# maua-maua-maua/maua

Hardware: AMD Instinct MI355X
Metric: frames/sec (whole node), 1024x1024 StyleGAN2 audio-reactive render (higher is better)
Workload: dtype bf16

## Files before the change

maua_amd/csrc/internal.h:

```cpp
#pragma once
#include "common.h"

namespace maua {

int launch_pack_rgb8(hipStream_t stream, const float* img, uint8_t* out, int B, int H, int W);
template <typename TI, typename TO>
int launch_nchw_to_nhwc(hipStream_t s, const void* x, void* y, int N, int C, int HW, int Cp);
template <typename TI, typename TO>
int launch_nhwc_to_nchw(hipStream_t s, const void* x, void* y, int N, int C, int HW, int Cp);

struct ConvArgs {
  const void* x;
  long x_bstride;
  const void* w;
  const float* s;
  const float* d;
  const float* noise;
  long noise_bstride;
  float noise_strength;
  const float* noise_scale;
  const float* bias;
  void* y;
  int B, H, W, Ci, Co, up;
  int act;
// ... 80 lines not shown
size_t upwalk_weight_elems(int Co, int Ci);
int launch_upwalk(hipStream_t stream, const HiresArgs& a, int dtype = MAUA_BF16);
int launch_prep_upwalk_weights(hipStream_t stream, const float* w, void* wt, int Co, int Ci, int flip, int dtype = MAUA_BF16);
bool upwalk_fused_supported(int dtype, int Ci, int Cm, int H, int W);
int launch_upwalk_fused(hipStream_t stream, const HiresArgs& up, const HiresArgs& c1, int force_segs = 0, int narrow_ok = 1,
                        int dtype = MAUA_BF16);

int launch_prep_weights(hipStream_t stream, int dtype, const float* w, void* wt, float* wsq, int Co, int Ci, int k,
                        int up, int flip, int Cop, int Cip);
int launch_f32_split_inplace(hipStream_t stream, void* w, long n_floats);

int launch_tconv2(hipStream_t stream, int dtype, const ConvArgs& a);
bool tconv_dma_supported(int dtype, int Ci, int Co, int H, int W);
int launch_tconv_dma(hipStream_t stream, const ConvArgs& a, int dtype = MAUA_BF16);
int launch_tconv_edges(hipStream_t stream, const ConvArgs& a, int dtype = MAUA_BF16);
int launch_prep_tconv_weights(hipStream_t stream, int dtype, const float* w, void* wt, int Co, int Ci, int flip);

struct UpfirArgs {
  const void* t;
  void* y;
  const float* d;
  const float* noise;
  long noise_bstride;
  float noise_strength;
  const float* noise_scale;
  const float* bias;
  const float* out_scale;
  int B, H, W, Co;
  int act;
  float alpha, gain, clamp;
};
int launch_upfir_epilogue(hipStream_t stream, int dtype, const UpfirArgs& a);
bool tconv_fir_supported(int dtype, int Ci, int Co, int H, int W);
int launch_tconv_fir(hipStream_t stream, const ConvArgs& a, const UpfirArgs& u, int dtype = MAUA_BF16);
size_t prepped_weight_elems(int k, int up, int Cop, int Cip);

struct LayerOperands { const void* x; const void* w; const float* s; const float* d; const float* bias; void* y; int B, H, W, Ci, Co, up; };
struct NoiseOperands { const float* noise; long bstride; float strength; const float* scale; };
struct Epilogue { int act; float alpha, gain, clamp; };
template <typename A>
inline void set_noise_args(A& a, const NoiseOperands& n) {
  a.noise = n.noise; a.noise_bstride = n.bstride; a.noise_strength = n.strength; a.noise_scale = n.scale;
}
template <typename A>
inline void set_epilogue_args(A& a, const Epilogue& e) {
  a.act = e.act; a.alpha = e.alpha; a.gain = e.gain; a.clamp = e.clamp;
}
template <typename A>
inline A layer_args(A a, const LayerOperands& l, const NoiseOperands& n, const Epilogue& e) {
  a.x = l.x; a.w = l.w; a.s = l.s; a.d = l.d; a.bias = l.bias; a.y = l.y;
  a.B = l.B; a.H = l.H; a.W = l.W; a.Ci = l.Ci; a.Co = l.Co; a.up = l.up;
  set_noise_args(a, n);
  set_epilogue_args(a, e);
  return a;
}
template <typename A>
inline void fuse_torgb_args(A& a, const float* wmod, const float* bias, const float* prev, float* out, float clamp, const float* fir16) {
  a.rgb_wmod = wmod; a.rgb_bias = bias; a.rgb_prev = prev; a.rgb_out = out; a.rgb_clamp = clamp;
  for (int i = 0; i < 16; i++) a.fir[i] = fir16[i];
}
inline void pack_u8_args(HiresArgs& a, uint8_t* rgb8_out, bool skip_f32) {
  a.rgb8_out = rgb8_out;
  a.rgb_skip_f32 = skip_f32;
}
inline ConvArgs tconv_args(const void* x, long x_bstride, const void* w, const float* s, void* t, int B, int H, int W, int Ci, int Co) {
  ConvArgs a{};
  a.x = x; a.x_bstride = x_bstride; a.w = w; a.s = s; a.y = t;
  a.B = B; a.H = H; a.W = W; a.Ci = Ci; a.Co = Co; a.up = 2;
  return a;
}
inline UpfirArgs upfir_args(void* y, const float* d, const float* bias, const float* out_scale, int B, int H, int W, int Co,
                            const NoiseOperands& n, const Epilogue& e) {
  UpfirArgs u{};
  u.y = y; u.d = d; u.bias = bias; u.out_scale = out_scale; u.B = B; u.H = H; u.W = W; u.Co = Co;
  set_noise_args(u, n);
  set_epilogue_args(u, e);
  return u;
}
inline void upsample_fir16(float* fir) {
  const float g4[4] = {0.25f, 0.75f, 0.75f, 0.25f};
  for (int u = 0; u < 4; u++)
    for (int v = 0; v < 4; v++) fir[u * 4 + v] = g4[u] * g4[v];
}

int modconv3x3_check(int dtype, const ConvArgs& a);
int lowres_check(int dtype, const ConvArgs& a);
int lowres_ksplit(int dtype, int B, int H, int W, int Ci, int Co, int up);
int hires_check(const HiresArgs& a, int dtype);
int upwalk_check(const HiresArgs& a, int dtype);
int upwalk_fused_check(const HiresArgs& up, const HiresArgs& c1, int dtype);
int tconv2_check(int dtype, const ConvArgs& a);
int tconv_edges_check(const ConvArgs& a, int dtype);
int tconv_dma_check(const ConvArgs& a, int dtype);
int tconv_fir_check(const ConvArgs& a, const UpfirArgs& u, int dtype);
int upfir_check(int dtype, const UpfirArgs& a);

struct ResizeArgs {
  const void* x;
  long x_bstride;
  void* y;
  int B, H, W, C, oh, ow;
  int mode;
  int align;
  int pl, pt;
  int how;
  float value;
  const float* noise;
};
int launch_resize2d(hipStream_t stream, int dtype, bool nhwc, const ResizeArgs& a);
int launch_skip_add(hipStream_t stream, const float* y, const float* prev, float* out, int B, int H, int W,
                    const float* fir16);
int launch_warp_affine_nhwc(hipStream_t stream, int dtype, const void* x, void* y, const float* minv, int B, int H, int W,
                            int C);

struct StyleLayer {
  const float* affine_w;
  const float* affine_b;
  const float* wsq;
  const float* wrgb;
  float* s;
  float* d;
  float* wmod;
  int w_index;
  int Cin, Co, Cs, Cd;
  float scale;
};
int launch_styles(hipStream_t stream, const StyleLayer* layers_dev, int n_layers, const float* ws, int num_ws,
// ... 172 lines not shown
```

maua_amd/csrc/modconv_api.hip:

```cpp
#include <algorithm>
#include <cstring>

#include "common.h"
#include "internal.h"

namespace maua {
namespace {

enum { R_LOWRES = 0, R_GENERIC, R_DMA, R_HIRES, R_UPWALK, R_FUSED, R_WALKDONE, R_TFIR, R_TDMA, R_T2, R_UPFIR };

bool is_tconv(int r) { return r == R_TFIR || r == R_TDMA || r == R_T2; }
bool reads_premod(int r) { return r == R_TFIR || r == R_TDMA || r == R_DMA; }

LayerOperands operands(const maua_modconv_desc* d) {
  return LayerOperands{d->x, nullptr, d->s, d->d, d->bias, d->y, d->B, d->H, d->W, d->Ci, d->Co, d->up};
}
NoiseOperands noise_of(const maua_modconv_desc* d) { return NoiseOperands{d->noise, d->noise_bstride, d->noise_strength, d->noise_scale}; }
Epilogue epilogue_of(const maua_modconv_desc* d) { return Epilogue{d->act, d->alpha, d->gain, d->clamp}; }

template <typename A>
A desc_args(const maua_modconv_desc* d) {
  A a = layer_args(A{}, operands(d), noise_of(d), epilogue_of(d));
  if (d->rgb_out) {
    float fir[16];
// ... 160 lines not shown
    MAUA_HIP_CHECK(hipGetLastError());
  }
  switch (route) {
    case R_LOWRES:
    case R_GENERIC:
    case R_DMA: {
      ConvArgs a = conv_args(d);
      a.x = x; a.x_bstride = x_bstride; a.w = base + o_w;
      if (route == R_DMA) a.s = nullptr;
      return route == R_LOWRES    ? launch_modconv_lowres(st, dtype, a, base + o_xm, (float*)(base + o_ws))
             : route == R_GENERIC ? launch_modconv3x3(st, dtype, a)
                                  : launch_modconv_dma(st, a, dtype);
    }
    case R_HIRES:
    case R_UPWALK:
    case R_FUSED: {
      HiresArgs a = hires_args(d);
      a.w = base + o_w;
      if (route == R_HIRES) return launch_modconv_hires(st, a, dtype);
      if (route == R_UPWALK) return launch_upwalk(st, a, dtype);
      HiresArgs f = hires_args(d1);
      f.x = nullptr; f.y = nullptr; f.w = base + o_w1;
      a.y = nullptr;
      return launch_upwalk_fused(st, a, f, force_segs, narrow_ok, dtype);
    }
    case R_TFIR:
    case R_TDMA:
    case R_T2: {
      void* t = d->t ? d->t : base + o_t;
      ConvArgs a = tconv_args(d);
      a.x = x; a.x_bstride = x_bstride; a.w = base + o_w; a.y = t;
      if (route != R_T2) a.s = (const float*)(base + o_ones);
      UpfirArgs u = upfir_args(d);
      if (route == R_TFIR) return launch_tconv_fir(st, a, u, dtype);
      if (route == R_TDMA) {
        if (int rc = launch_tconv_edges(st, a, dtype)) return rc;
        if (int rc = launch_tconv_dma(st, a, dtype)) return rc;
      } else if (int rc = launch_tconv2(st, dtype, a)) {
        return rc;
      }
      u.t = t;
      return launch_upfir_epilogue(st, dtype, u);
    }
    case R_UPFIR: {
      UpfirArgs u = upfir_args(d);
      u.t = d->x;
      return launch_upfir_epilogue(st, dtype, u);
    }
  }
  return MAUA_OK;
}

extern "C" int maua_torgb_ex(maua_ctx* ctx, const void* x, const float* wmod, const float* bias, const float* prev, float* out, int B,
                             int H, int W, int C, float clamp, int dtype) {
  MAUA_REQUIRE(ctx && x && wmod && bias && out, "maua_torgb_ex: NULL argument");
  MAUA_REQUIRE(B >= 0 && H > 0 && W > 0 && C > 0, "maua_torgb_ex: bad shape");
  MAUA_REQUIRE(!prev || (H % 2 == 0 && W % 2 == 0), "maua_torgb_ex: the skip image needs an even grid");
  RgbArgs r{};
  r.x = x; r.wmod = wmod; r.bias = bias; r.prev = prev; r.out = out; r.B = B; r.H = H; r.W = W; r.C = C; r.clamp = clamp;
  upsample_fir16(r.fir);
  return launch_torgb(ctx->stream, dtype, r);
}
```

maua_amd/csrc/modconv_tconv_fir.hip:

```cpp
#include "common.h"
#include "internal.h"

namespace maua {

namespace {

constexpr int PTW = 32;
constexpr int HW1 = PTW + 1;
constexpr int KB = 64;
constexpr int WROWS = 9 * 32;
constexpr int WBUF = WROWS * KB;
constexpr int OFF_H = 2 * WBUF;
constexpr int ES = 128 * 2;

__device__ __constant__ const int kSlotF[9] = {0, 1, 1, 2, 2, 3, 3, 3, 3};
__device__ __constant__ const int kClsF[9] = {0, 0, 1, 0, 2, 0, 1, 2, 3};

__device__ __forceinline__ unsigned lds_off(const void* p) {
  return (unsigned)(size_t)(__attribute__((address_space(3))) const void*)p;
}
__device__ __forceinline__ void dma16_s(const void* sbase, unsigned voff, unsigned lds_dst) {
  asm volatile("s_mov_b32 m0, %2\n\ts_nop 0\n\tglobal_load_lds_dwordx4 %0, %1" ::"v"(voff), "s"(sbase), "s"(lds_dst)
               : "memory");
}
template <typename F>
__device__ __forceinline__ void mma(f32x16& acc, const u32x4& w, const u32x4& x) {
  Mma16<F>::step(acc, w, x);
}
__device__ __forceinline__ int swz(int n) { return (n >> 2) & 3; }

__device__ __forceinline__ int t_col(int tc, int pc) {
  const int p = tc >> 1;
  return p * ES + ((((tc & 1) ^ (p & 3)) << 6) | ((pc ^ ((p >> 2) & 3)) << 4));
}

template <typename F>
__device__ __forceinline__ void fir_hrow(const char* tile, int tr, const int (&tcol)[5], f32x2_t (&h)[2][4]) {
  f32x2_t c[5][4];
  const int rowb = (tr >> 1) * (PTW * ES), rsw = (tr & 1) << 7;
#pragma unroll
  for (int rx = 0; rx < 5; rx++) {
    const u32x4 v = *reinterpret_cast<const u32x4*>(tile + rowb + (tcol[rx] ^ rsw));
#pragma unroll
    for (int k = 0; k < 4; k++) c[rx][k] = f32x2_t{Fmt16<F>::lo(v[k]), Fmt16<F>::hi(v[k])};
  }
#pragma unroll
  for (int e = 0; e < 4; e++) {
    h[0][e] = (c[0][e] + c[3][e]) + 3.f * (c[1][e] + c[2][e]);
    h[1][e] = (c[1][e] + c[4][e]) + 3.f * (c[2][e] + c[3][e]);
  }
}

}

template <int PTH_, typename F>
__global__ __launch_bounds__(PTH_ * 32, PTH_ == 8 ? 2 : 1) void tconv_fir_kernel(ConvArgs a, UpfirArgs u) {
  constexpr int PTH = PTH_, UPR = PTH - 2;
  constexpr int HPX = (PTH + 1) * HW1, HBUF = HPX * KB;
  constexpr int NW = PTH / 2, NT = NW * 64;
  constexpr int WJ = (WBUF / 1024 + NW - 1) / NW, HJ = (HPX * 4 + NT - 1) / NT;
  constexpr int FG = NT / 128, FROWS = 2 * UPR / FG;
  static_assert(FG * FROWS == 2 * UPR, "output rows must split evenly over the FIR groups");
  extern __shared__ __attribute__((aligned(1024))) char smem[];
  const unsigned lds0 = __builtin_amdgcn_readfirstlane(lds_off(smem));
  const int tid = threadIdx.x, lane = tid & 63;
  const int wave = __builtin_amdgcn_readfirstlane(tid >> 6);
  const int r = lane & 31, h = lane >> 5;
  const int tiles_x = (a.W + 29) / 30, tiles = tiles_x * ((a.H + UPR - 1) / UPR), CB = a.Co >> 5;
  const int cbg = CB < 8 ? CB : 8, n_ts = tiles * a.B, per_group = ((n_ts + 7) >> 3) * 8 * cbg;
  const int L = blockIdx.x, grp = L / per_group, Lg = L - grp * per_group;
  const int xcd = Lg & 7, idx = Lg >> 3;
  const int cb = grp * cbg + idx % cbg, ts = (idx / cbg) * 8 + xcd;
  if (ts >= n_ts) return;
  const int b = ts / tiles, tile = ts - b * tiles;
  const int tyi = tile / tiles_x, txi = tile - tyi * tiles_x;
  const int ty0 = tyi * UPR - 1, tx0 = txi * 30 - 1;
  const char* xb = reinterpret_cast<const char*>(a.x) + (long)b * a.x_bstride * 2;
  const char* wp = reinterpret_cast<const char*>(a.w);

  unsigned hoff[HJ];
#pragma unroll
  for (int j = 0; j < HJ; j++) {
    const int P = (wave + NW * j) * 64 + lane;
    const int hp = P >> 2, q = (P & 3) ^ swz(hp);
    const int py = (hp * 1986) >> 16;
    const int px = hp - py * HW1;
    const int gy = ty0 - 1 + py, gx = tx0 - 1 + px;
    hoff[j] = 0xffffffffu;
    if (P < HPX * 4) {
      if (gy >= 0 && gx >= 0 && gy < a.H && gx < a.W) {
        hoff[j] = (unsigned)(((gy * a.W + gx) * a.Ci + q * 8) * 2);
      } else {
        *reinterpret_cast<u32x4*>(smem + OFF_H + P * 16) = u32x4{0u, 0u, 0u, 0u};
        *reinterpret_cast<u32x4*>(smem + OFF_H + HBUF + P * 16) = u32x4{0u, 0u, 0u, 0u};
      }
    }
  }
  unsigned woff[WJ];
#pragma unroll
  for (int j = 0; j < WJ; j++) {
    const int ii = wave + NW * j;
    const int R = min(16 * ii + (lane >> 2), WROWS - 1);
    const int k = R >> 5, n = R & 31;
    const int q = (lane & 3) ^ swz(R);
    woff[j] = (unsigned)((((((kSlotF[k] * CB + cb) * 4 + kClsF[k]) * 32 + n) * a.Ci) + q * 8) * 2);
  }
#define TD_ISSUE(C_, BUF_)                                                                               \
  {                                                                                                      \
    const char* ws_ = wp + (long)(C_) * KB;                                                              \
    _Pragma("unroll") for (int j = 0; j < WJ; j++)                                                      \
      if (wave + NW * j < WBUF / 1024) dma16_s(ws_, woff[j], lds0 + (BUF_) * WBUF + (wave + NW * j) * 1024); \
    const char* xs_ = xb + (long)(C_) * KB;                                                              \
    _Pragma("unroll") for (int j = 0; j < HJ; j++)                                                      \
      if (hoff[j] != 0xffffffffu) dma16_s(xs_, hoff[j], lds0 + OFF_H + (BUF_) * HBUF + (wave + NW * j) * 1024); \
  }

  const int hp00 = (2 * wave) * HW1 + r;
  const unsigned b0 = (unsigned)(r * KB + ((swz(r) ^ h) << 4));
#define TD_A(HR_, Q1_, KS_, BUF_)                                                                        \
  ({                                                                                                     \
    const int hp_ = hpv + (HR_) * HW1 + (Q1_);                                                           \
    *reinterpret_cast<const u32x4*>(smem + ((OFF_H + (BUF_) * HBUF + hp_ * KB + ((swz(hp_) ^ h) << 4)) ^ ((KS_) << 5))); \
  })
#define TD_B(K_, KS_, BUF_) (*reinterpret_cast<const u32x4*>(smem + (BUF_) * WBUF + (K_) * 32 * KB + (b0 ^ ((KS_) << 5))))

  f32x16 acc[2][4];
#pragma unroll
  for (int R = 0; R < 2; R++)
#pragma unroll
    for (int c = 0; c < 4; c++)
#pragma unroll
      for (int e = 0; e < 16; e++) acc[R][c][e] = 0.f;

  const int n_chunks = a.Ci >> 5;
  TD_ISSUE(0, 0)
  if (n_chunks > 1) TD_ISSUE(1, 1)
  asm volatile("s_waitcnt vmcnt(0)" ::: "memory");
  __syncthreads();
  int hpv = hp00;
#define TD_STEP(KS_, BUF_)                                                                               \
  {                                                                                                      \
    u32x4 A00 = TD_A(0, 0, KS_, BUF_), A01 = TD_A(0, 1, KS_, BUF_);      \
    u32x4 A10 = TD_A(1, 0, KS_, BUF_), A11 = TD_A(1, 1, KS_, BUF_);                    \
    u32x4 A20 = TD_A(2, 0, KS_, BUF_), A21 = TD_A(2, 1, KS_, BUF_);                    \
    {                                                                                                    \
      const u32x4 B0 = TD_B(0, KS_, BUF_), B1 = TD_B(1, KS_, BUF_), B2 = TD_B(2, KS_, BUF_);              \
      mma<F>(acc[0][0], B0, A00); mma<F>(acc[1][0], B0, A10);                                 \
      mma<F>(acc[0][1], B2, A01); mma<F>(acc[1][1], B2, A11);                        \
      mma<F>(acc[0][0], B1, A01); mma<F>(acc[1][0], B1, A11);                        \
    }                                                                                                    \
    {                                                                                                    \
      const u32x4 B3 = TD_B(3, KS_, BUF_), B4 = TD_B(4, KS_, BUF_);                                       \
      mma<F>(acc[0][2], B4, A10); mma<F>(acc[1][2], B4, A20);                        \
      mma<F>(acc[0][0], B3, A10); mma<F>(acc[1][0], B3, A20);                        \
    }                                                                                                    \
    {                                                                                                    \
      const u32x4 B5 = TD_B(5, KS_, BUF_), B6 = TD_B(6, KS_, BUF_), B7 = TD_B(7, KS_, BUF_), B8 = TD_B(8, KS_, BUF_); \
      mma<F>(acc[0][3], B8, A11); mma<F>(acc[1][3], B8, A21);                                 \
      mma<F>(acc[0][1], B6, A11); mma<F>(acc[1][1], B6, A21);                                                  \
      mma<F>(acc[0][2], B7, A11); mma<F>(acc[1][2], B7, A21);                                                  \
      mma<F>(acc[0][0], B5, A11); mma<F>(acc[1][0], B5, A21);                                                  \
    }                                                                                                    \
  }
  for (int c = 0; c < n_chunks; c++) {
    const int buf = c & 1;
    asm volatile("" : "+v"(hpv));
    TD_STEP(0, buf)
    {
      u32x4 A00 = TD_A(0, 0, 1, buf), A01 = TD_A(0, 1, 1, buf), A10 = TD_A(1, 0, 1, buf), A11 = TD_A(1, 1, 1, buf);
      u32x4 A20 = TD_A(2, 0, 1, buf), A21 = TD_A(2, 1, 1, buf);
      const u32x4 B0 = TD_B(0, 1, buf), B1 = TD_B(1, 1, buf), B2 = TD_B(2, 1, buf), B3 = TD_B(3, 1, buf), B4 = TD_B(4, 1, buf);
      const u32x4 B5 = TD_B(5, 1, buf), B6 = TD_B(6, 1, buf), B7 = TD_B(7, 1, buf), B8 = TD_B(8, 1, buf);
      asm volatile("s_waitcnt vmcnt(0)" ::: "memory");
      __syncthreads();
      if (c + 2 < n_chunks) TD_ISSUE(c + 2, buf)
      mma<F>(acc[0][0], B0, A00); mma<F>(acc[1][0], B0, A10);
      mma<F>(acc[0][1], B2, A01); mma<F>(acc[1][1], B2, A11);
      mma<F>(acc[0][0], B1, A01); mma<F>(acc[1][0], B1, A11);
      mma<F>(acc[0][2], B4, A10); mma<F>(acc[1][2], B4, A20);
      mma<F>(acc[0][0], B3, A10); mma<F>(acc[1][0], B3, A20);
      mma<F>(acc[0][3], B8, A11); mma<F>(acc[1][3], B8, A21);
      mma<F>(acc[0][1], B6, A11); mma<F>(acc[1][1], B6, A21);
      mma<F>(acc[0][2], B7, A11); mma<F>(acc[1][2], B7, A21);
      mma<F>(acc[0][0], B5, A11); mma<F>(acc[1][0], B5, A21);
    }
  }
#undef TD_ISSUE
#undef TD_A
#undef TD_B
#undef TD_STEP

  const int fhalf = tid / 120, fw = tid - fhalf * 120;
  const int strip = fw >> 2, pc = fw & 3;
  const int xl = 2 + 2 * strip, yl0 = 2 + FROWS * fhalf;
  const int X = 2 * tx0 + xl, Wo = 2 * a.W, Ho = 2 * a.H;
  const int cho = cb * 32 + pc * 8;
  const bool fir_on = tid < 120 * FG && X < Wo;
  f32x2_t dv[4], bv[4], sv[4];
  float2 nzv[FROWS];
#pragma unroll
  for (int k = 0; k < FROWS; k++) nzv[k] = make_float2(0.f, 0.f);
  if (fir_on) {
#pragma unroll
    for (int e4 = 0; e4 < 8; e4 += 4) {
      const float4 s4 = u.out_scale ? *reinterpret_cast<const float4*>(u.out_scale + (long)b * a.Co + cho + e4)
                                    : make_float4(1.f, 1.f, 1.f, 1.f);
      sv[e4 / 2] = f32x2_t{s4.x, s4.y}; sv[e4 / 2 + 1] = f32x2_t{s4.z, s4.w};
      const float4 d4 = u.d ? *reinterpret_cast<const float4*>(u.d + (long)b * a.Co + cho + e4) : make_float4(1.f, 1.f, 1.f, 1.f);
      const float4 b4 = u.bias ? *reinterpret_cast<const float4*>(u.bias + cho + e4) : make_float4(0.f, 0.f, 0.f, 0.f);
      dv[e4 / 2] = f32x2_t{d4.x, d4.y}; dv[e4 / 2 + 1] = f32x2_t{d4.z, d4.w};
      bv[e4 / 2] = f32x2_t{b4.x, b4.y}; bv[e4 / 2 + 1] = f32x2_t{b4.z, b4.w};
    }
    if (u.noise) {
      const float* nb = u.noise + (long)b * u.noise_bstride;
#pragma unroll
      for (int k = 0; k < FROWS; k++) {
        const int Y = 2 * ty0 + yl0 + k;
        if (Y < Ho) nzv[k] = *reinterpret_cast<const float2*>(nb + (long)Y * Wo + X);
      }
    }
  }
  __syncthreads();
  char* tt = smem;
#pragma unroll
  for (int R = 0; R < 2; R++) {
    const int m = (2 * wave + R) * 32 + r;
#pragma unroll
    for (int c = 0; c < 4; c++)
#pragma unroll
      for (int qd = 0; qd < 4; qd++)
        *reinterpret_cast<uint2*>(tt + m * ES + (((c ^ (r & 3)) << 6) | ((qd ^ ((r >> 2) & 3)) << 4) | (h << 3))) =
            make_uint2(Fmt16<F>::pack2(acc[R][c][qd * 4 + 0], acc[R][c][qd * 4 + 1]), Fmt16<F>::pack2(acc[R][c][qd * 4 + 2], acc[R][c][qd * 4 + 3]));
  }
  __syncthreads();
  {
    if (fir_on) {
#pragma unroll
      for (int e = 0; e < 4; e++) { dv[e] *= 0.0625f * u.gain; bv[e] *= u.gain; }
      const float nzs = u.noise_strength * u.gain * (u.noise_scale ? u.noise_scale[b] : 1.f);
      const float cl = u.clamp >= 0.f ? u.clamp : 3.0e38f;
      char* yb = reinterpret_cast<char*>(u.y) + (long)b * Ho * Wo * a.Co * 2;
      int tcol[5];
#pragma unroll
      for (int rx = 0; rx < 5; rx++) tcol[rx] = t_col(xl - 1 + rx, pc);
      f32x2_t hr[4][2][4];
      fir_hrow<F>(tt, yl0 - 1, tcol, hr[0]);
      fir_hrow<F>(tt, yl0, tcol, hr[1]);
      fir_hrow<F>(tt, yl0 + 1, tcol, hr[2]);
#pragma unroll
      for (int k = 0; k < FROWS; k++) {
        fir_hrow<F>(tt, yl0 + k + 2, tcol, hr[(k + 3) & 3]);
        const int Y = 2 * ty0 + yl0 + k;
        if (Y < Ho) {
          const float nz[2] = {nzv[k].x * nzs, nzv[k].y * nzs};
#pragma unroll
          for (int j = 0; j < 2; j++) {
            f32x2_t o[4];
#pragma unroll
            for (int e = 0; e < 4; e++) {
              const f32x2_t accv = (hr[k & 3][j][e] + hr[(k + 3) & 3][j][e]) + 3.f * (hr[(k + 1) & 3][j][e] + hr[(k + 2) & 3][j][e]);
              f32x2_t t = accv * dv[e] + (bv[e] + nz[j]);
              const f32x2_t ta = t * u.alpha;
              t = f32x2_t{fmaxf(t[0], ta[0]), fmaxf(t[1], ta[1])};
              o[e] = f32x2_t{__builtin_amdgcn_fmed3f(t[0], -cl, cl), __builtin_amdgcn_fmed3f(t[1], -cl, cl)} * sv[e];
            }
            *reinterpret_cast<u32x4*>(yb + (((long)Y * Wo + X + j) * a.Co + cho) * 2) =
                u32x4{Fmt16<F>::pack2(o[0][0], o[0][1]), Fmt16<F>::pack2(o[1][0], o[1][1]), Fmt16<F>::pack2(o[2][0], o[2][1]), Fmt16<F>::pack2(o[3][0], o[3][1])};
          }
        }
      }
    }
  }
}

bool tconv_fir_supported(int dtype, int Ci, int Co, int H, int W) {
  return (dtype == MAUA_BF16 || dtype == MAUA_F16) && Ci % 32 == 0 && Co % 32 == 0 && H >= 16 && W >= 32 && (long)H * W * Ci * 2 < (1L << 32) &&
         16L * Co * Ci * 2 < (1L << 32);
}

int tconv_fir_check(const ConvArgs& a, const UpfirArgs& u, int dtype) {
  MAUA_REQUIRE(tconv_fir_supported(dtype, a.Ci, a.Co, a.H, a.W), "tconv_fir: unsupported shape");
  MAUA_REQUIRE(u.act == MAUA_ACT_LRELU && u.alpha >= 0.f && u.alpha <= 1.f && u.gain > 0.f, "tconv_fir: lrelu epilogue only");
  MAUA_REQUIRE(!u.noise || (((uintptr_t)u.noise % 8) == 0 && u.noise_bstride % 2 == 0), "tconv_fir: noise must be 8-byte aligned");
  const int pth = 8, upr = pth - 2;
  const int tiles = ((a.H + upr - 1) / upr) * ((a.W + 29) / 30), CB = a.Co / 32, cbg = CB < 8 ? CB : 8;
  MAUA_REQUIRE(CB % cbg == 0, "tconv_fir: channel blocks must split into groups of 8");
  const long n_ts = (long)tiles * a.B, grid = ((n_ts + 7) / 8) * 8 * cbg * (CB / cbg);
  MAUA_REQUIRE(grid < (1L << 31), "tconv_fir: grid too large");
  return MAUA_OK;
}

int launch_tconv_fir(hipStream_t stream, const ConvArgs& a, const UpfirArgs& u, int dtype) {
  if (int rc = tconv_fir_check(a, u, dtype)) return rc;
  if (a.B == 0) return MAUA_OK;
  const int pth = 8, upr = pth - 2;
  const int tiles = ((a.H + upr - 1) / upr) * ((a.W + 29) / 30), CB = a.Co / 32, cbg = CB < 8 ? CB : 8;
  const long n_ts = (long)tiles * a.B, grid = ((n_ts + 7) / 8) * 8 * cbg * (CB / cbg);
  const size_t smem = std::max<size_t>((size_t)2 * WBUF + 2 * (pth + 1) * HW1 * KB, (size_t)pth * PTW * ES);
  if (dtype == MAUA_F16) {
    MAUA_HIP_CHECK(hipFuncSetAttribute((const void*)tconv_fir_kernel<8, f16_t>, hipFuncAttributeMaxDynamicSharedMemorySize, (int)smem));
    hipLaunchKernelGGL((tconv_fir_kernel<8, f16_t>), dim3((unsigned)grid), dim3(256), smem, stream, a, u);
  } else {
    MAUA_HIP_CHECK(hipFuncSetAttribute((const void*)tconv_fir_kernel<8, bf16_t>, hipFuncAttributeMaxDynamicSharedMemorySize, (int)smem));
    hipLaunchKernelGGL((tconv_fir_kernel<8, bf16_t>), dim3((unsigned)grid), dim3(256), smem, stream, a, u);
  }
  MAUA_HIP_CHECK(hipGetLastError());
  return MAUA_OK;
}

}
```

maua_amd/csrc/synth.hip:

```cpp
#include <cmath>
#include <cstring>
#include <string>
#include <vector>

#include "common.h"
#include "internal.h"

using namespace maua;

namespace {

struct ConvLayer {
  int block, which;
  int Ci, Co, res, up, w_index;
  int ih = 0, iw = 0;
  int oh = 0, ow = 0;
  int fh = 0, fw = 0;
  float* affine_w = nullptr;
  float* affine_b = nullptr;
  float* bias = nullptr;
  float* noise_const = nullptr;
  float noise_strength = 0.f;
  void* wt = nullptr;
  void* wt_t = nullptr;
// ... 9 lines not shown
  float* affine_w = nullptr;
  float* affine_b = nullptr;
  float* wrgb = nullptr;
  float* bias = nullptr;
  float* s = nullptr;
  float* wmod = nullptr;
};

template <typename T>
int dev_alloc(T** p, size_t n) {
  MAUA_HIP_CHECK(hipMalloc((void**)p, n * sizeof(T)));
  return MAUA_OK;
}

}

struct maua_synth {
  maua_ctx* ctx;
  int res, w_dim, channel_base, channel_max, dtype, nv_compat;
  int nblocks, num_ws;
  size_t esize;
  std::vector<ConvLayer> convs;
  std::vector<RgbLayer> rgbs;
  void* const_x = nullptr;
  int keep_features = 0;
  int lowres = 1;
  int use_hires = 1;
  int upwalk = 2;
  int walk_segs = 0;
  int walk_narrow = 1;
  int fuse_torgb = 1;
  int tconv_up = 1;
  int tconv_fir = 256;
  const float* nz_scales = nullptr;
  long nz_scale_stride = 0;
  int dma_conv = 1;
  int dual_store = 1;
  int tconv_dma = 1;
  float* ones = nullptr;
  void* xm = nullptr;
  void* tbuf = nullptr;
  void* lowres_xm = nullptr;
  float* lowres_ws = nullptr;
  int rs_layer = -1, rs_mode = 0, rs_th = 0, rs_tw = 0, rs_pl = 0, rs_pr = 0, rs_pt = 0, rs_pb = 0, rs_how = 3;
  float rs_value = 0.f;
  float* rs_noise = nullptr;
  void* const_rs = nullptr;
  float* rgb_tmp[2] = {nullptr, nullptr};
  int out_h = 0, out_w = 0;
  int warp_layer[3] = {-1, -1, -1};
  const float* warp_minv[3] = {nullptr, nullptr, nullptr};
  int profile = 0;
  std::vector<hipEvent_t> ev;
  size_t ev_used = 0;
  std::vector<size_t> ev_fwd_start;
  int bcap = 0;
  void* act[2] = {nullptr, nullptr};
  float* img[2] = {nullptr, nullptr};
  StyleLayer* style_table_dev = nullptr;
  float fir[16];
};

static void prof_mark(maua_synth* n) {
  if (!n->profile || n->ev_used >= (1u << 16)) return;
  if (n->ev_used == n->ev.size()) {
    hipEvent_t e;
// ... 402 lines not shown
  n->warp_layer[slot] = inv_matrices_dev ? layer : -1;
  n->warp_minv[slot] = inv_matrices_dev;
  return MAUA_OK;
}

int maua_synth_layer_size(const maua_synth* n, int layer, int* h, int* w) {
  MAUA_REQUIRE(n && h && w, "maua_synth_layer_size: NULL argument");
  MAUA_REQUIRE(layer >= -1 && layer < (int)n->convs.size(), "maua_synth_layer_size: no such layer");
  if (layer < 0) { *h = n->out_h; *w = n->out_w; }
  else { *h = n->convs[layer].oh; *w = n->convs[layer].ow; }
  return MAUA_OK;
}

int maua_synth_set_option(maua_synth* n, const char* key, int value) {
  MAUA_REQUIRE(n && key, "maua_synth_set_option: NULL argument");
  if (!strcmp(key, "profile")) {
    n->profile = value;
    n->ev_used = 0;
    n->ev_fwd_start.clear();
    return MAUA_OK;
  }
  if (!strcmp(key, "keep_features")) {
    if (n->keep_features != value) {
      MAUA_HIP_CHECK(hipStreamSynchronize(n->ctx->stream));
      free_workspace(n);
      n->keep_features = value;
    }
    return MAUA_OK;
  }
  static const std::pair<const char*, int maua_synth::*> routing[] = {
      {"lowres", &maua_synth::lowres},         {"use_hires", &maua_synth::use_hires}, {"upwalk", &maua_synth::upwalk},
      {"walk_segs", &maua_synth::walk_segs},   {"walk_narrow", &maua_synth::walk_narrow},
      {"fuse_torgb", &maua_synth::fuse_torgb}, {"tconv_up", &maua_synth::tconv_up},   {"tconv_fir", &maua_synth::tconv_fir},
      {"tconv_dma", &maua_synth::tconv_dma},   {"dma_conv", &maua_synth::dma_conv},   {"dual_store", &maua_synth::dual_store}};
  for (const auto& o : routing)
    if (!strcmp(key, o.first)) {
      n->*o.second = value;
      return MAUA_OK;
    }
  return fail(std::string("maua_synth_set_option: unknown option ") + key);
}

static thread_local hipMemcpyKind g_load_kind = hipMemcpyHostToDevice;

static int upload(float* dst, const float* host, size_t count, size_t expect, const char* name) {
  if (count != expect)
    return fail(std::string("maua_synth_load: ") + name + ": expected " + std::to_string(expect) + " values, got " +
                std::to_string(count));
  MAUA_HIP_CHECK(hipMemcpy(dst, host, count * sizeof(float), g_load_kind));
  return MAUA_OK;
}

int maua_synth_load(maua_synth* n, const char* name, const float* host, size_t count) {
  MAUA_REQUIRE(n && name && host, "maua_synth_load: NULL argument");
  std::string s(name);
  int blk = -1, pos = 0;
  if (sscanf(name, "bs.%d.%n", &blk, &pos) < 1 || blk < 0 || blk >= n->nblocks || pos == 0)
    return fail("maua_synth_load: unknown parameter name: " + s);
  std::string rest = s.substr(pos);
  hipStream_t st = n->ctx->stream;
  auto check_filter = [&]() -> int {
    if (count != 16) return fail("maua_synth_load: " + s + ": only the 4x4 [1,3,3,1] resample filter is supported");
    const float t[4] = {1, 3, 3, 1};
    for (int u = 0; u < 4; u++)
      for (int v = 0; v < 4; v++)
        if (std::fabs(host[u * 4 + v] - t[u] * t[v] / 64.f) > 1e-6f)
// ... 155 lines not shown
        }
        case Route::Hires:
        case Route::Upwalk:
        case Route::FusedWalk: {
          HiresArgs a = layer_args(HiresArgs{}, li, x, s.skip_store ? nullptr : y);
          if (s.rgb) fuse_torgb(a);
          if (s.rgb8) pack_u8(a);
          if (s.route != Route::Hires) a.w = c.wt_h;
          if (s.route != Route::FusedWalk) {
            if (int rc = s.route == Route::Hires ? launch_modconv_hires(st, a, n->dtype) : launch_upwalk(st, a, n->dtype)) return rc;
            break;
          }
          HiresArgs f = layer_args(HiresArgs{}, li + 1, nullptr, nullptr);
          fuse_torgb(f);
          if (plan.conv[li + 1].rgb8) pack_u8(f);
          if (int rc = launch_upwalk_fused(st, a, f, n->walk_segs, n->walk_narrow, n->dtype)) return rc;
          break;
        }
        case Route::WalkDone:
          break;
        case Route::TconvFir:
        case Route::TconvDma:
        case Route::Tconv2: {
          ConvArgs a = tconv_args(x, x_bstride, c.wt_t, c.s, n->tbuf, B, c.ih, c.iw, c.Ci, c.Co);
          UpfirArgs u = upfir_args(y, c.d, c.bias, next_s, B, c.ih, c.iw, c.Co, layer_noise(li), lrelu_epilogue());
          if (s.src == Src::PremodPass)
            if (int rc = launch_premod_nhwc(st, x, x_bstride, c.s, n->xm, B, (long)c.ih * c.iw, c.Ci, n->dtype)) return rc;
          if (s.src == Src::PremodPass || s.src == Src::Xm) {
            a.x = n->xm;
            a.x_bstride = (long)c.ih * c.iw * c.Ci;
          }
          if (reads_premod(s.route)) a.s = n->ones;
          if (s.route == Route::TconvFir) {
            if (int rc = launch_tconv_fir(st, a, u, n->dtype)) return rc;
            prof_mark(n);
            break;
          }
          if (s.route == Route::TconvDma) {
            if (int rc = launch_tconv_edges(st, a, n->dtype)) return rc;
            if (int rc = launch_tconv_dma(st, a, n->dtype)) return rc;
          } else if (int rc = launch_tconv2(st, n->dtype, a)) {
            return rc;
          }
          prof_mark(n);
          u.t = n->tbuf;
          if (int rc = launch_upfir_epilogue(st, n->dtype, u)) return rc;
          break;
        }
      }
      prof_mark(n);
      x = y;
      x_bstride = (long)c.oh * c.ow * c.Co;
      cur ^= 1;
      if (hooked) {
        void* dst = n->keep_features ? c.feat : n->act[cur];
        if (int rc = resize_feat(x, x_bstride, B, c.oh, c.ow, c.Co, dst)) return rc;
        x = dst;
        x_bstride = (long)c.fh * c.fw * c.Co;
        cur ^= 1;
      }
      for (int wsl = 0; wsl < 3; wsl++) {
        if (n->warp_layer[wsl] != (int)li + 1 || !n->warp_minv[wsl]) continue;
        void* dst = n->act[cur];
        if (dst == x) dst = n->act[cur ^ 1];
        if (int rc = launch_warp_affine_nhwc(st, n->dtype, x, dst, n->warp_minv[wsl], B, c.fh, c.fw, c.Co)) return rc;
        if (n->keep_features) {
          MAUA_HIP_CHECK(hipMemcpyAsync(c.feat, dst, (size_t)B * c.fh * c.fw * c.Co * n->esize, hipMemcpyDeviceToDevice, st));
// ... 111 lines not shown
```

Baseline: 4583.

## Walk vertical segments of tiles in tconv_fir, carrying halo rows across tiles

The fused transposed-conv + FIR kernel now processes a vertical segment of up to 8 row tiles per block instead of a single 8-row tile with 2 halo rows recomputed per tile. The last three t rows are carried in registers into a dedicated LDS carry region, so the next tile's FIR can reuse them and the overlapping conv rows are not recomputed. Weight offsets are hoisted out of the tile loop. This adds a segment-length option, fewer but longer-running blocks that may reduce parallelism on small layers, and an extra barrier per tile.

```diff
diff --git a/maua_amd/csrc/internal.h b/maua_amd/csrc/internal.h
--- a/maua_amd/csrc/internal.h
+++ b/maua_amd/csrc/internal.h
@@ -136,7 +136,8 @@
 };
 int launch_upfir_epilogue(hipStream_t stream, int dtype, const UpfirArgs& a);
 bool tconv_fir_supported(int dtype, int Ci, int Co, int H, int W);
-int launch_tconv_fir(hipStream_t stream, const ConvArgs& a, const UpfirArgs& u, int dtype = MAUA_BF16);
+int tconv_fir_seg_tiles(int H, int W);
+int launch_tconv_fir(hipStream_t stream, const ConvArgs& a, const UpfirArgs& u, int dtype = MAUA_BF16, int seg_tiles = 0);
 size_t prepped_weight_elems(int k, int up, int Cop, int Cip);
 
 struct LayerOperands { const void* x; const void* w; const float* s; const float* d; const float* bias; void* y; int B, H, W, Ci, Co, up; };
@@ -196,7 +197,7 @@
 int tconv2_check(int dtype, const ConvArgs& a);
 int tconv_edges_check(const ConvArgs& a, int dtype);
 int tconv_dma_check(const ConvArgs& a, int dtype);
-int tconv_fir_check(const ConvArgs& a, const UpfirArgs& u, int dtype);
+int tconv_fir_check(const ConvArgs& a, const UpfirArgs& u, int dtype, int seg_tiles = 0);
 int upfir_check(int dtype, const UpfirArgs& a);
 
 struct ResizeArgs {
diff --git a/maua_amd/csrc/modconv_api.hip b/maua_amd/csrc/modconv_api.hip
--- a/maua_amd/csrc/modconv_api.hip
+++ b/maua_amd/csrc/modconv_api.hip
@@ -216,7 +216,7 @@
       a.x = x; a.x_bstride = x_bstride; a.w = base + o_w; a.y = t;
       if (route != R_T2) a.s = (const float*)(base + o_ones);
       UpfirArgs u = upfir_args(d);
-      if (route == R_TFIR) return launch_tconv_fir(st, a, u, dtype);
+      if (route == R_TFIR) return launch_tconv_fir(st, a, u, dtype, force_segs);
       if (route == R_TDMA) {
         if (int rc = launch_tconv_edges(st, a, dtype)) return rc;
         if (int rc = launch_tconv_dma(st, a, dtype)) return rc;
diff --git a/maua_amd/csrc/modconv_tconv_fir.hip b/maua_amd/csrc/modconv_tconv_fir.hip
--- a/maua_amd/csrc/modconv_tconv_fir.hip
+++ b/maua_amd/csrc/modconv_tconv_fir.hip
@@ -12,6 +12,9 @@
 constexpr int WBUF = WROWS * KB;
 constexpr int OFF_H = 2 * WBUF;
 constexpr int ES = 128 * 2;
+constexpr int TROW = 64 * 32 * 2;
+constexpr int OFF_C = 8 * PTW * ES;
+constexpr int TF_LDS = OFF_C + 3 * TROW;
 
 __device__ __constant__ const int kSlotF[9] = {0, 1, 1, 2, 2, 3, 3, 3, 3};
 __device__ __constant__ const int kClsF[9] = {0, 0, 1, 0, 2, 0, 1, 2, 3};
@@ -34,13 +37,14 @@
   return p * ES + ((((tc & 1) ^ (p & 3)) << 6) | ((pc ^ ((p >> 2) & 3)) << 4));
 }
 
+__device__ __forceinline__ int c_col(int tcol) { return ((tcol >> 8) << 7) | ((tcol ^ ((tcol >> 1) & 0x40)) & 0x7f); }
+
 template <typename F>
-__device__ __forceinline__ void fir_hrow(const char* tile, int tr, const int (&tcol)[5], f32x2_t (&h)[2][4]) {
+__device__ __forceinline__ void fir_hrow(const char* row, int rsw, const int (&col)[5], f32x2_t (&h)[2][4]) {
   f32x2_t c[5][4];
-  const int rowb = (tr >> 1) * (PTW * ES), rsw = (tr & 1) << 7;
 #pragma unroll
   for (int rx = 0; rx < 5; rx++) {
-    const u32x4 v = *reinterpret_cast<const u32x4*>(tile + rowb + (tcol[rx] ^ rsw));
+    const u32x4 v = *reinterpret_cast<const u32x4*>(row + (col[rx] ^ rsw));
 #pragma unroll
     for (int k = 0; k < 4; k++) c[rx][k] = f32x2_t{Fmt16<F>::lo(v[k]), Fmt16<F>::hi(v[k])};
   }
@@ -54,19 +58,20 @@
 }
 
 template <int PTH_, typename F>
-__global__ __launch_bounds__(PTH_ * 32, PTH_ == 8 ? 2 : 1) void tconv_fir_kernel(ConvArgs a, UpfirArgs u) {
-  constexpr int PTH = PTH_, UPR = PTH - 2;
+__global__ __launch_bounds__(PTH_ * 32, 2) void tconv_fir_kernel(ConvArgs a, UpfirArgs u, int seg_n) {
+  static_assert(PTH_ == 8, "the segment walk is written for 8-row tiles");
+  constexpr int PTH = PTH_;
   constexpr int HPX = (PTH + 1) * HW1, HBUF = HPX * KB;
   constexpr int NW = PTH / 2, NT = NW * 64;
   constexpr int WJ = (WBUF / 1024 + NW - 1) / NW, HJ = (HPX * 4 + NT - 1) / NT;
-  constexpr int FG = NT / 128, FROWS = 2 * UPR / FG;
-  static_assert(FG * FROWS == 2 * UPR, "output rows must split evenly over the FIR groups");
+  constexpr int FMAX = 8;
   extern __shared__ __attribute__((aligned(1024))) char smem[];
   const unsigned lds0 = __builtin_amdgcn_readfirstlane(lds_off(smem));
   const int tid = threadIdx.x, lane = tid & 63;
   const int wave = __builtin_amdgcn_readfirstlane(tid >> 6);
   const int r = lane & 31, h = lane >> 5;
-  const int tiles_x = (a.W + 29) / 30, tiles = tiles_x * ((a.H + UPR - 1) / UPR), CB = a.Co >> 5;
+  const int seg_rows = 8 * seg_n - 2;
+  const int tiles_x = (a.W + 29) / 30, tiles = tiles_x * ((a.H + seg_rows - 1) / seg_rows), CB = a.Co >> 5;
   const int cbg = CB < 8 ? CB : 8, n_ts = tiles * a.B, per_group = ((n_ts + 7) >> 3) * 8 * cbg;
   const int L = blockIdx.x, grp = L / per_group, Lg = L - grp * per_group;
   const int xcd = Lg & 7, idx = Lg >> 3;
@@ -74,14 +79,37 @@
   if (ts >= n_ts) return;
   const int b = ts / tiles, tile = ts - b * tiles;
   const int tyi = tile / tiles_x, txi = tile - tyi * tiles_x;
-  const int ty0 = tyi * UPR - 1, tx0 = txi * 30 - 1;
+  const int sy0 = tyi * seg_rows, tx0 = txi * 30 - 1;
+  const int n_tiles = min(seg_n, (a.H - sy0 + 9) >> 3);
   const char* xb = reinterpret_cast<const char*>(a.x) + (long)b * a.x_bstride * 2;
   const char* wp = reinterpret_cast<const char*>(a.w);
 
+  unsigned woff[WJ];
+#pragma unroll
+  for (int j = 0; j < WJ; j++) {
+    const int ii = wave + NW * j;
+    const int R = min(16 * ii + (lane >> 2), WROWS - 1);
+    const int k = R >> 5, n = R & 31;
+    const int q = (lane & 3) ^ swz(R);
+    woff[j] = (unsigned)((((((kSlotF[k] * CB + cb) * 4 + kClsF[k]) * 32 + n) * a.Ci) + q * 8) * 2);
+  }
+  const int hp00 = (2 * wave) * HW1 + r;
+  const unsigned b0 = (unsigned)(r * KB + ((swz(r) ^ h) << 4));
+  const int Wo = 2 * a.W, Ho = 2 * a.H;
+  const int n_chunks = a.Ci >> 5;
+  char* tt = smem;
+  u32x4 carry[3];
+#pragma unroll
+  for (int i = 0; i < 3; i++) carry[i] = u32x4{0u, 0u, 0u, 0u};
+
+  for (int tk = 0; tk < n_tiles; tk++) {
+  const int ty0 = sy0 - 1 + 8 * tk;
   unsigned hoff[HJ];
+  int hl = lane;
+  asm volatile("" : "+v"(hl));
 #pragma unroll
   for (int j = 0; j < HJ; j++) {
-    const int P = (wave + NW * j) * 64 + lane;
+    const int P = (wave + NW * j) * 64 + hl;
     const int hp = P >> 2, q = (P & 3) ^ swz(hp);
     const int py = (hp * 1986) >> 16;
     const int px = hp - py * HW1;
@@ -96,15 +124,6 @@
       }
     }
   }
-  unsigned woff[WJ];
-#pragma unroll
-  for (int j = 0; j < WJ; j++) {
-    const int ii = wave + NW * j;
-    const int R = min(16 * ii + (lane >> 2), WROWS - 1);
-    const int k = R >> 5, n = R & 31;
-    const int q = (lane & 3) ^ swz(R);
-    woff[j] = (unsigned)((((((kSlotF[k] * CB + cb) * 4 + kClsF[k]) * 32 + n) * a.Ci) + q * 8) * 2);
-  }
 #define TD_ISSUE(C_, BUF_)                                                                               \
   {                                                                                                      \
     const char* ws_ = wp + (long)(C_) * KB;                                                              \
@@ -115,8 +134,6 @@
       if (hoff[j] != 0xffffffffu) dma16_s(xs_, hoff[j], lds0 + OFF_H + (BUF_) * HBUF + (wave + NW * j) * 1024); \
   }
 
-  const int hp00 = (2 * wave) * HW1 + r;
-  const unsigned b0 = (unsigned)(r * KB + ((swz(r) ^ h) << 4));
 #define TD_A(HR_, Q1_, KS_, BUF_)                                                                        \
   ({                                                                                                     \
     const int hp_ = hpv + (HR_) * HW1 + (Q1_);                                                           \
@@ -132,10 +149,9 @@
 #pragma unroll
       for (int e = 0; e < 16; e++) acc[R][c][e] = 0.f;
 
-  const int n_chunks = a.Ci >> 5;
   TD_ISSUE(0, 0)
   if (n_chunks > 1) TD_ISSUE(1, 1)
-  asm volatile("s_waitcnt vmcnt(0)" ::: "memory");
+  __builtin_amdgcn_s_waitcnt(0x0f70);
   __syncthreads();
   int hpv = hp00;
 #define TD_STEP(KS_, BUF_)                                                                               \
@@ -190,16 +206,23 @@
 #undef TD_B
 #undef TD_STEP
 
-  const int fhalf = tid / 120, fw = tid - fhalf * 120;
+  int ft = tid;
+  float fzero = 0.f, gain = u.gain, clampv = u.clamp;
+  asm volatile("" : "+v"(ft), "+v"(fzero), "+s"(gain), "+s"(clampv));
+  const int fr = ft & 31, fh = (ft >> 5) & 1;
+  const int fhalf = ft / 120, fw = ft - fhalf * 120;
   const int strip = fw >> 2, pc = fw & 3;
-  const int xl = 2 + 2 * strip, yl0 = 2 + FROWS * fhalf;
-  const int X = 2 * tx0 + xl, Wo = 2 * a.W, Ho = 2 * a.H;
+  const int xl = 2 + 2 * strip;
+  const int X = 2 * tx0 + xl;
   const int cho = cb * 32 + pc * 8;
-  const bool fir_on = tid < 120 * FG && X < Wo;
+  const bool fir_on = ft < 240 && X < Wo;
+  const int g0 = tk == 0 ? 1 + 6 * fhalf : 8 * fhalf - 3;
+  const int frows = tk == 0 ? 6 : 8;
+  const int Y0 = 2 * ty0 + g0 + 1;
   f32x2_t dv[4], bv[4], sv[4];
-  float2 nzv[FROWS];
-#pragma unroll
-  for (int k = 0; k < FROWS; k++) nzv[k] = make_float2(0.f, 0.f);
+  float2 nzv[FMAX];
+#pragma unroll
+  for (int k = 0; k < FMAX; k++) nzv[k] = make_float2(fzero, fzero);
   if (fir_on) {
 #pragma unroll
     for (int e4 = 0; e4 < 8; e4 += 4) {
@@ -214,63 +237,84 @@
     if (u.noise) {
       const float* nb = u.noise + (long)b * u.noise_bstride;
 #pragma unroll
-      for (int k = 0; k < FROWS; k++) {
-        const int Y = 2 * ty0 + yl0 + k;
-        if (Y < Ho) nzv[k] = *reinterpret_cast<const float2*>(nb + (long)Y * Wo + X);
+      for (int k = 0; k < FMAX; k++) {
+        const int Y = Y0 + k;
+        if (k < frows && Y < Ho) nzv[k] = *reinterpret_cast<const float2*>(nb + (long)Y * Wo + X);
       }
     }
   }
   __syncthreads();
-  char* tt = smem;
 #pragma unroll
   for (int R = 0; R < 2; R++) {
-    const int m = (2 * wave + R) * 32 + r;
+    const int m = (2 * wave + R) * 32 + fr;
 #pragma unroll
     for (int c = 0; c < 4; c++)
 #pragma unroll
       for (int qd = 0; qd < 4; qd++)
-        *reinterpret_cast<uint2*>(tt + m * ES + (((c ^ (r & 3)) << 6) | ((qd ^ ((r >> 2) & 3)) << 4) | (h << 3))) =
+        *reinterpret_cast<uint2*>(tt + m * ES + (((c ^ (fr & 3)) << 6) | ((qd ^ ((fr >> 2) & 3)) << 4) | (fh << 3))) =
             make_uint2(Fmt16<F>::pack2(acc[R][c][qd * 4 + 0], acc[R][c][qd * 4 + 1]), Fmt16<F>::pack2(acc[R][c][qd * 4 + 2], acc[R][c][qd * 4 + 3]));
+  }
+  const int ccol = t_col(ft >> 2, ft & 3);
+  if (tk > 0) {
+#pragma unroll
+    for (int i = 0; i < 3; i++) *reinterpret_cast<u32x4*>(smem + OFF_C + i * TROW + c_col(ccol)) = carry[i];
   }
   __syncthreads();
   {
     if (fir_on) {
 #pragma unroll
-      for (int e = 0; e < 4; e++) { dv[e] *= 0.0625f * u.gain; bv[e] *= u.gain; }
-      const float nzs = u.noise_strength * u.gain * (u.noise_scale ? u.noise_scale[b] : 1.f);
-      const float cl = u.clamp >= 0.f ? u.clamp : 3.0e38f;
+      for (int e = 0; e < 4; e++) { dv[e] *= 0.0625f * gain; bv[e] *= gain; }
+      const float nzs = u.noise_strength * gain * (u.noise_scale ? u.noise_scale[b] : 1.f);
+      const float cl = clampv >= 0.f ? clampv : 3.0e38f;
       char* yb = reinterpret_cast<char*>(u.y) + (long)b * Ho * Wo * a.Co * 2;
       int tcol[5];
 #pragma unroll
       for (int rx = 0; rx < 5; rx++) tcol[rx] = t_col(xl - 1 + rx, pc);
       f32x2_t hr[4][2][4];
-      fir_hrow<F>(tt, yl0 - 1, tcol, hr[0]);
-      fir_hrow<F>(tt, yl0, tcol, hr[1]);
-      fir_hrow<F>(tt, yl0 + 1, tcol, hr[2]);
-#pragma unroll
-      for (int k = 0; k < FROWS; k++) {
-        fir_hrow<F>(tt, yl0 + k + 2, tcol, hr[(k + 3) & 3]);
-        const int Y = 2 * ty0 + yl0 + k;
-        if (Y < Ho) {
-          const float nz[2] = {nzv[k].x * nzs, nzv[k].y * nzs};
-#pragma unroll
-          for (int j = 0; j < 2; j++) {
-            f32x2_t o[4];
-#pragma unroll
-            for (int e = 0; e < 4; e++) {
-              const f32x2_t accv = (hr[k & 3][j][e] + hr[(k + 3) & 3][j][e]) + 3.f * (hr[(k + 1) & 3][j][e] + hr[(k + 2) & 3][j][e]);
-              f32x2_t t = accv * dv[e] + (bv[e] + nz[j]);
-              const f32x2_t ta = t * u.alpha;
-              t = f32x2_t{fmaxf(t[0], ta[0]), fmaxf(t[1], ta[1])};
-              o[e] = f32x2_t{__builtin_amdgcn_fmed3f(t[0], -cl, cl), __builtin_amdgcn_fmed3f(t[1], -cl, cl)} * sv[e];
+      if (g0 < 0) {
+        int cc[5];
+#pragma unroll
+        for (int rx = 0; rx < 5; rx++) cc[rx] = c_col(tcol[rx]);
+#pragma unroll
+        for (int i = 0; i < 3; i++) fir_hrow<F>(smem + OFF_C + i * TROW, 0, cc, hr[i]);
+      } else {
+#pragma unroll
+        for (int i = 0; i < 3; i++) fir_hrow<F>(tt + ((g0 + i) >> 1) * (PTW * ES), ((g0 + i) & 1) << 7, tcol, hr[i]);
+      }
+#pragma unroll
+      for (int k = 0; k < FMAX; k++) {
+        if (k < frows) {
+          const int g = g0 + k + 3;
+          fir_hrow<F>(tt + (g >> 1) * (PTW * ES), (g & 1) << 7, tcol, hr[(k + 3) & 3]);
+          const int Y = Y0 + k;
+          if (Y < Ho) {
+            const float nz[2] = {nzv[k].x * nzs, nzv[k].y * nzs};
+#pragma unroll
+            for (int j = 0; j < 2; j++) {
+              f32x2_t o[4];
+#pragma unroll
+              for (int e = 0; e < 4; e++) {
+                const f32x2_t accv = (hr[k & 3][j][e] + hr[(k + 3) & 3][j][e]) + 3.f * (hr[(k + 1) & 3][j][e] + hr[(k + 2) & 3][j][e]);
+                f32x2_t t = accv * dv[e] + (bv[e] + nz[j]);
+                const f32x2_t ta = t * u.alpha;
+                t = f32x2_t{fmaxf(t[0], ta[0]), fmaxf(t[1], ta[1])};
+                o[e] = f32x2_t{__builtin_amdgcn_fmed3f(t[0], -cl, cl), __builtin_amdgcn_fmed3f(t[1], -cl, cl)} * sv[e];
+              }
+              *reinterpret_cast<u32x4*>(yb + (((long)Y * Wo + X + j) * a.Co + cho) * 2) =
+                  u32x4{Fmt16<F>::pack2(o[0][0], o[0][1]), Fmt16<F>::pack2(o[1][0], o[1][1]), Fmt16<F>::pack2(o[2][0], o[2][1]), Fmt16<F>::pack2(o[3][0], o[3][1])};
             }
-            *reinterpret_cast<u32x4*>(yb + (((long)Y * Wo + X + j) * a.Co + cho) * 2) =
-                u32x4{Fmt16<F>::pack2(o[0][0], o[0][1]), Fmt16<F>::pack2(o[1][0], o[1][1]), Fmt16<F>::pack2(o[2][0], o[2][1]), Fmt16<F>::pack2(o[3][0], o[3][1])};
           }
         }
       }
     }
   }
+  if (tk + 1 < n_tiles) {
+    carry[0] = *reinterpret_cast<const u32x4*>(tt + 6 * (PTW * ES) + (ccol ^ 128));
+    carry[1] = *reinterpret_cast<const u32x4*>(tt + 7 * (PTW * ES) + ccol);
+    carry[2] = *reinterpret_cast<const u32x4*>(tt + 7 * (PTW * ES) + (ccol ^ 128));
+    __syncthreads();
+  }
+  }
 }
 
 bool tconv_fir_supported(int dtype, int Ci, int Co, int H, int W) {
@@ -278,31 +322,46 @@
          16L * Co * Ci * 2 < (1L << 32);
 }
 
-int tconv_fir_check(const ConvArgs& a, const UpfirArgs& u, int dtype) {
+int tconv_fir_seg_tiles(int H, int W) {
+  (void)W;
+  const int whole = (H + 2 + 7) / 8;
+  return whole < 8 ? whole : 8;
+}
+
+namespace {
+constexpr int kMaxSegTiles = 4096;
+long tconv_fir_grid(const ConvArgs& a, int seg) {
+  const int seg_rows = 8 * seg - 2;
+  const int tiles = ((a.H + seg_rows - 1) / seg_rows) * ((a.W + 29) / 30), CB = a.Co / 32, cbg = CB < 8 ? CB : 8;
+  const long n_ts = (long)tiles * a.B;
+  return ((n_ts + 7) / 8) * 8 * cbg * (CB / cbg);
+}
+}
+
+int tconv_fir_check(const ConvArgs& a, const UpfirArgs& u, int dtype, int seg_tiles) {
   MAUA_REQUIRE(tconv_fir_supported(dtype, a.Ci, a.Co, a.H, a.W), "tconv_fir: unsupported shape");
   MAUA_REQUIRE(u.act == MAUA_ACT_LRELU && u.alpha >= 0.f && u.alpha <= 1.f && u.gain > 0.f, "tconv_fir: lrelu epilogue only");
   MAUA_REQUIRE(!u.noise || (((uintptr_t)u.noise % 8) == 0 && u.noise_bstride % 2 == 0), "tconv_fir: noise must be 8-byte aligned");
-  const int pth = 8, upr = pth - 2;
-  const int tiles = ((a.H + upr - 1) / upr) * ((a.W + 29) / 30), CB = a.Co / 32, cbg = CB < 8 ? CB : 8;
+  MAUA_REQUIRE(seg_tiles >= 0 && seg_tiles <= kMaxSegTiles, "tconv_fir: tiles per segment out of range");
+  const int CB = a.Co / 32, cbg = CB < 8 ? CB : 8;
   MAUA_REQUIRE(CB % cbg == 0, "tconv_fir: channel blocks must split into groups of 8");
-  const long n_ts = (long)tiles * a.B, grid = ((n_ts + 7) / 8) * 8 * cbg * (CB / cbg);
-  MAUA_REQUIRE(grid < (1L << 31), "tconv_fir: grid too large");
+  MAUA_REQUIRE(tconv_fir_grid(a, seg_tiles ? seg_tiles : tconv_fir_seg_tiles(a.H, a.W)) < (1L << 31), "tconv_fir: grid too large");
   return MAUA_OK;
 }
 
-int launch_tconv_fir(hipStream_t stream, const ConvArgs& a, const UpfirArgs& u, int dtype) {
-  if (int rc = tconv_fir_check(a, u, dtype)) return rc;
+int launch_tconv_fir(hipStream_t stream, const ConvArgs& a, const UpfirArgs& u, int dtype, int seg_tiles) {
+  if (int rc = tconv_fir_check(a, u, dtype, seg_tiles)) return rc;
   if (a.B == 0) return MAUA_OK;
-  const int pth = 8, upr = pth - 2;
-  const int tiles = ((a.H + upr - 1) / upr) * ((a.W + 29) / 30), CB = a.Co / 32, cbg = CB < 8 ? CB : 8;
-  const long n_ts = (long)tiles * a.B, grid = ((n_ts + 7) / 8) * 8 * cbg * (CB / cbg);
-  const size_t smem = std::max<size_t>((size_t)2 * WBUF + 2 * (pth + 1) * HW1 * KB, (size_t)pth * PTW * ES);
+  const int seg = seg_tiles ? seg_tiles : tconv_fir_seg_tiles(a.H, a.W);
+  const long grid = tconv_fir_grid(a, seg);
+  static_assert(TF_LDS >= 2 * WBUF + 2 * 9 * HW1 * KB, "the t tile and its carry alias the K buffers");
+  const size_t smem = TF_LDS;
   if (dtype == MAUA_F16) {
     MAUA_HIP_CHECK(hipFuncSetAttribute((const void*)tconv_fir_kernel<8, f16_t>, hipFuncAttributeMaxDynamicSharedMemorySize, (int)smem));
-    hipLaunchKernelGGL((tconv_fir_kernel<8, f16_t>), dim3((unsigned)grid), dim3(256), smem, stream, a, u);
+    hipLaunchKernelGGL((tconv_fir_kernel<8, f16_t>), dim3((unsigned)grid), dim3(256), smem, stream, a, u, seg);
   } else {
     MAUA_HIP_CHECK(hipFuncSetAttribute((const void*)tconv_fir_kernel<8, bf16_t>, hipFuncAttributeMaxDynamicSharedMemorySize, (int)smem));
-    hipLaunchKernelGGL((tconv_fir_kernel<8, bf16_t>), dim3((unsigned)grid), dim3(256), smem, stream, a, u);
+    hipLaunchKernelGGL((tconv_fir_kernel<8, bf16_t>), dim3((unsigned)grid), dim3(256), smem, stream, a, u, seg);
   }
   MAUA_HIP_CHECK(hipGetLastError());
   return MAUA_OK;
diff --git a/maua_amd/csrc/synth.hip b/maua_amd/csrc/synth.hip
--- a/maua_amd/csrc/synth.hip
+++ b/maua_amd/csrc/synth.hip
@@ -65,6 +65,7 @@
   int fuse_torgb = 1;
   int tconv_up = 1;
   int tconv_fir = 256;
+  int tconv_fir_seg = 0;
   const float* nz_scales = nullptr;
   long nz_scale_stride = 0;
   int dma_conv = 1;
@@ -533,6 +534,7 @@
       {"lowres", &maua_synth::lowres},         {"use_hires", &maua_synth::use_hires}, {"upwalk", &maua_synth::upwalk},
       {"walk_segs", &maua_synth::walk_segs},   {"walk_narrow", &maua_synth::walk_narrow},
       {"fuse_torgb", &maua_synth::fuse_torgb}, {"tconv_up", &maua_synth::tconv_up},   {"tconv_fir", &maua_synth::tconv_fir},
+      {"tconv_fir_seg", &maua_synth::tconv_fir_seg},
       {"tconv_dma", &maua_synth::tconv_dma},   {"dma_conv", &maua_synth::dma_conv},   {"dual_store", &maua_synth::dual_store}};
   for (const auto& o : routing)
     if (!strcmp(key, o.first)) {
@@ -754,7 +756,7 @@
           }
           if (reads_premod(s.route)) a.s = n->ones;
           if (s.route == Route::TconvFir) {
-            if (int rc = launch_tconv_fir(st, a, u, n->dtype)) return rc;
+            if (int rc = launch_tconv_fir(st, a, u, n->dtype, n->tconv_fir_seg)) return rc;
             prof_mark(n);
             break;
           }
```

Result: no change. 4625 (median of 6 runs) (+0.9%).
